# neyuru/RayTracing

Measured on AMD Instinct MI355X. Metric: ray-steps/sec (whole node) on vert_heterogeneous, 1M rays; % HBM roofline, higher is better.
Workload: dtype f64

## Files before the change

raytracing_amd/csrc/rtmi.hip:

```cpp
#include <hip/hip_runtime.h>

#include <chrono>
#include <cmath>
#include <cstdio>
#include <cstdlib>
#include <algorithm>
#include <cstring>
#include <exception>
#include <mutex>
#include <numeric>
#include <new>
#include <string>
#include <thread>
#include <utility>
#include <vector>

#include "rt_device.h"
#include "rtmi_field.h"

static thread_local std::string g_err;
static int fail(int code, const std::string& msg) {
    g_err = msg;
    return code;
}
// ... 212 lines not shown
template <typename T> __device__ __forceinline__ void derive_rt(const BatchDev<T>& a, rt::Ray<T>& r) {
    if (a.iso) rt::derive<T, true>(a.K, r); else rt::derive<T, false>(a.K, r);
}
template <> __device__ __forceinline__ void derive_rt<double>(const BatchDev<double>& a, rt::Ray<double>& r) {
    if (a.exact) rt::ex::derive(a.K, r);
    else if (a.iso) rt::derive<double, true>(a.K, r);
    else rt::derive<double, false>(a.K, r);
}
template <typename T> using InitGather = rt::PolyGather<T, rt::kPolyLane>;
template <typename T> __device__ __forceinline__ void n_gradient_rt(const BatchDev<T>& a, T x, T y, T& n, T& gx, T& gy) {
    InitGather<T> gg;
    rt::n_gradient(a.F, gg, true, x, y, n, gx, gy);
}
template <> __device__ __forceinline__ void n_gradient_rt<double>(const BatchDev<double>& a, double x, double y, double& n, double& gx, double& gy) {
    if (a.exact) { rt::GlobalGather<double> gg; rt::ex::n_gradient(a.F, gg, true, x, y, n, gx, gy); }
    else { InitGather<double> gg; rt::n_gradient(a.F, gg, true, x, y, n, gx, gy); }
}

template <typename T> __device__ __forceinline__ void init_ray(const BatchDev<T>& a, long k) {
    rt::Ray<T> r;
    r.x = a.x0[k]; r.y = a.y0[k]; r.th = a.th0[k];
    n_gradient_rt(a, (T)r.x, (T)r.y, r.n, r.gx, r.gy);
    derive_rt(a, r);
    r.dsim = 0; r.dreal = 0; r.tt = 0;
    a.acc(0)[k] = r.x; a.acc(1)[k] = r.y; a.acc(2)[k] = r.th; a.aux(0)[k] = r.n; a.aux(1)[k] = r.gx; a.aux(2)[k] = r.gy;
    a.acc(3)[k] = 0; a.acc(4)[k] = 0; a.acc(5)[k] = 0;
    if (a.has_hist) { a.aux(3)[k] = 0; a.aux(4)[k] = 0; a.aux(5)[k] = 0; a.aux(6)[k] = 0; }
    if (a.rot) { a.unit(0)[k] = r.ux; a.unit(1)[k] = r.uy; }
    if (a.hov) a.hov[k] = 0.f;
    a.istep[k] = 0;
    a.alive[k] = max_size_of(a, k) > 1;
    if (a.stride && a.rec_rows > 0) write_row(a, 0, k, r);
}
template <typename T> __global__ void k_init(BatchDev<T> a) {
    const long k = (long)blockIdx.x * blockDim.x + threadIdx.x;
    if (k >= a.R) return;
    init_ray(a, k);
}

__device__ __forceinline__ unsigned long long wave_sum(unsigned long long v) {
#pragma unroll
    for (int o = 32; o > 0; o >>= 1) v += __shfl_xor(v, o, 64);
    return v;
}

__global__ void k_stats(const int* istep, const unsigned char* alive, long R, unsigned long long* counters) {
    unsigned long long steps = 0, live = 0;
    for (long k = (long)blockIdx.x * blockDim.x + threadIdx.x; k < R; k += (long)gridDim.x * blockDim.x) {
        steps += (unsigned long long)istep[k];
        live += alive[k];
    }
    steps = wave_sum(steps);
    live = wave_sum(live);
    if ((threadIdx.x & 63) == 0) {
        if (steps) atomicAdd(&counters[0], steps);
        if (live) atomicAdd(&counters[1], live);
    }
}

template <bool COH, typename V> __device__ __forceinline__ V ld_state(const V* p) {
    if constexpr (COH) return __hip_atomic_load(p, __ATOMIC_RELAXED, __HIP_MEMORY_SCOPE_AGENT);
    else return *p;
}
template <bool COH, typename V> __device__ __forceinline__ void st_state(V* p, V v) {
    if constexpr (COH) __hip_atomic_store(p, v, __ATOMIC_RELAXED, __HIP_MEMORY_SCOPE_AGENT);
    else *p = v;
}
template <typename T, int METHOD, bool ISO, bool COH = false, bool HOV = false>
__device__ __forceinline__ void load_ray(const BatchDev<T>& a, long k, rt::Ray<T>& r, int& i) {
    r.x = ld_state<COH>(a.acc(0) + k); r.y = ld_state<COH>(a.acc(1) + k); r.th = ld_state<COH>(a.acc(2) + k);
// ... 455 lines not shown
    int flavour = kOrdinary;
    int slot() const { return (iso ? 1 : 0) | (lds ? 2 : 0) | flat << 2 | flavour << 4; }
    bool operator==(const StepBuild& o) const { return dtype == o.dtype && ki == o.ki && slot() == o.slot(); }
};
struct rtmi_batch {
    const rtmi_field* field = nullptr;
    rtmi_params p{};
    int64_t R = 0;
    size_t esz = 8;
    hipStream_t stream = nullptr;
    void* state = nullptr;
    int* istep = nullptr;
    unsigned char* alive = nullptr;
    void *s_ray = nullptr, *n_ray = nullptr;
    bool own_s = false, own_n = false;
    double* launch = nullptr;
    int* perm = nullptr;
    void *vstep = nullptr, *vstep2h = nullptr;
    int* vmax = nullptr;
    unsigned long long* counters = nullptr;
    unsigned long long* h_counters = nullptr;
    std::vector<std::pair<hipEvent_t, hipEvent_t>> events;
    size_t ev_used = 0;
    size_t pass_ev_start = 0;
    double kernel_ms = 0;
    double total_kernel_ms = 0;
    uint64_t total_launches = 0;
    uint32_t launches = 0;
    int persistent_blocks = 0;
    int sliced_blocks = 0;
    unsigned long long* sliced_ctl = nullptr;
    bool dirty = false;
    bool dirty_state = false;
    bool state_rows = false;
    double auto_ms[2][RTMI_AUTO_SAMPLES] = {{0, 0, 0}, {0, 0, 0}};
    int auto_n[2] = {0, 0};
    int auto_kept = -1;
    double gold_sup[8] = {0, 0, 0, 0, 0, 0, 0, 0};
    int lat_simds = 0;
    int mode_used = RTMI_LAUNCH_PLAIN;
    const void* kfn_used = nullptr;
    uint32_t auto_fallbacks = 0;
    void* staging = nullptr;
    size_t staging_bytes = 0;
    hipGraph_t graph = nullptr;
    hipGraphExec_t graph_exec = nullptr;
    StepBuild graph_build;
    int graph_nsteps = 0, graph_count = 0, graph_block = 0;
    struct Retrace* rt = nullptr;
    bool is_retrace_sub = false;
};
static void drop_graph(rtmi_batch* b);

struct Retrace {
    rtmi_batch* sub = nullptr;
    unsigned cap = 0;
    unsigned long long* rq = nullptr;
    unsigned* host_count = nullptr;
    float* hov = nullptr;
    static constexpr int kAux = 4;
    hipStream_t aux[kAux] = {nullptr, nullptr, nullptr, nullptr};
    hipEvent_t ev_main = nullptr, ev_aux[kAux] = {nullptr, nullptr, nullptr, nullptr};
    hipStream_t masked = nullptr;
    hipEvent_t ev_in = nullptr, ev_out = nullptr;
    unsigned chunks = 0;
    unsigned launched = 0;
    unsigned scattered = 0;
    bool pending = false;
    unsigned long long* dbg = nullptr;
    unsigned overflow = 0;
    double* org = nullptr;
    int* org_istep = nullptr;
    bool from_set = false;
    unsigned swept = 0;
    uint64_t total = 0;
    unsigned rot = 0;
    bool rot_learned = false;
};
static int retrace_create(rtmi_batch* b, const double* x0, const double* y0, const double* theta0);
static void retrace_destroy(rtmi_batch* b);
static int retrace_reset(rtmi_batch* b);
static int retrace_drain(rtmi_batch* b, bool overlap);
static bool retrace_wanted(const rtmi_batch* b);
#define RETRACE_FLUSH(b)                                             \
    do {                                                             \
        if ((b)->rt && (b)->rt->pending) {                           \
            const int rcf_ = retrace_drain((b), false);              \
            if (rcf_) return rcf_;                                   \
        }                                                            \
    } while (0)

static int batch_staging(rtmi_batch* b, size_t bytes, void** out) {
    if (bytes > b->staging_bytes) {
        HIP_TRY(hipStreamSynchronize(b->stream));
        (void)hipFree(b->staging);
        b->staging = nullptr; b->staging_bytes = 0;
        hipError_t e = hipMalloc(&b->staging, bytes);
        if (e != hipSuccess) return fail(RTMI_ERR_ALLOC, std::string("staging buffer: ") + hipGetErrorString(e));
        b->staging_bytes = bytes;
    }
    *out = b->staging;
    return RTMI_OK;
}

constexpr long kWindowMinRays = 131072;
static bool window_loses(const rtmi_batch* b) {
    const int m = b->p.method;
    if (m != 5 && m != 9 && m != 10 && m != 11) return false;
    const rtmi_field* f = b->field;
    return std::fabs(b->p.step) > 0.5 * std::fmin(f->hx, f->hy);
}
template <typename T> static BatchDev<T> batch_dev(const rtmi_batch* b) {
    BatchDev<T> a;
    a.F = field_dev<T>(b->field, b->p.exact_basis);
    a.F.window = (b->p.field_path == 3 || (b->p.field_path == 0 && b->R >= kWindowMinRays && !window_loses(b))) ? 1 : 0;
    const rtmi_params& p = b->p;
    a.K.step = (T)p.step;
    a.K.step2h = (T)(libm_square(p.step) / 2.0);
    a.K.step2 = (T)libm_square(p.step);
    a.K.gamma = (T)p.gamma; a.K.g2m1 = (T)(p.gamma * p.gamma - 1.0);
    a.K.gamma_s = (T)p.gamma_step; a.K.g2m1_s = (T)(p.gamma_step * p.gamma_step - 1.0);
// ... 138 lines not shown
}

template <typename T, typename F> static hipError_t with_step_node_t(const rtmi_batch* b, const StepBuild& k, int sched, int nsteps, F&& use) {
    BatchDev<T> a = batch_dev<T>(b);
    int refill_min = b->p.refill_min > 0 ? b->p.refill_min : 32, chunk = 16;
    unsigned long long capacity = 0, timeout = 0, *ctl = b->sliced_ctl;
    void* plain[] = {&a, &nsteps};
    void* refill[] = {&a, &refill_min, &chunk};
    void* sliced[] = {&a, &nsteps, &capacity, &ctl, &timeout};
    const long bundles = (b->R + 255) / 256;
    hipKernelNodeParams kp{};
    kp.func = const_cast<void*>(step_kernel(k, sched));
    kp.blockDim = dim3(256);
    if (sched == RTMI_LAUNCH_PLAIN) {
        const int bs = b->p.block_size > 0 ? b->p.block_size : 256;
        kp.gridDim = dim3((unsigned)((b->R + bs - 1) / bs));
        kp.blockDim = dim3(bs);
        kp.kernelParams = plain;
    } else if (sched == RTMI_LAUNCH_SLICED) {
        capacity = sliced_capacity(b, nsteps);
        timeout = sliced_timeout_ticks(b, nsteps);
        kp.gridDim = dim3((unsigned)(bundles < b->sliced_blocks ? bundles : b->sliced_blocks));
        kp.kernelParams = sliced;
    } else {
        kp.gridDim = dim3((unsigned)(bundles < b->persistent_blocks ? bundles : b->persistent_blocks));
        kp.kernelParams = refill;
    }
    return use(kp);
}
template <typename F> static hipError_t with_step_node(const rtmi_batch* b, const StepBuild& k, int sched, int nsteps, F&& use) {
    return by_dtype(k.dtype, [&](auto t) { return with_step_node_t<decltype(t)>(b, k, sched, nsteps, use); });
}

static int batch_init_state(rtmi_batch* b, bool clear_traj) {
    hipStream_t st = b->stream;
    const size_t R = (size_t)b->R;
    HIP_TRY(hipMemsetAsync(b->counters, 0, 4 * sizeof(unsigned long long), st));
    if (b->rt) { const int rcr = retrace_reset(b); if (rcr) return rcr; }
    if (clear_traj && b->s_ray) HIP_TRY(hipMemsetAsync(b->s_ray, 0, (size_t)b->p.rec_rows * 6 * R * b->esz, st));
    if (clear_traj && b->n_ray) HIP_TRY(hipMemsetAsync(b->n_ray, 0, (size_t)b->p.rec_rows * R * b->esz, st));
    b->dirty = false;
    by_dtype(b->p.dtype, [&](auto t) { hipLaunchKernelGGL(k_init<decltype(t)>, blocks(b->R), dim3(256), 0, st, batch_dev<decltype(t)>(b)); });
    HIP_TRY(hipGetLastError());
    b->kernel_ms = 0; b->launches = 0; b->pass_ev_start = b->ev_used; b->dirty_state = false;
    b->state_rows = false;
    return RTMI_OK;
}

RTMI_EXPORT void rtmi_batch_destroy(rtmi_batch* b) {
    if (!b) return;
    (void)hipStreamSynchronize(b->stream);
    (void)hipFree(b->state); (void)hipFree(b->istep); (void)hipFree(b->alive); (void)hipFree(b->launch);
    (void)hipFree(b->perm);
    (void)hipFree(b->vstep); (void)hipFree(b->vstep2h); (void)hipFree(b->vmax);
    (void)hipFree(b->counters); (void)hipFree(b->sliced_ctl); (void)hipFree(b->staging);
    if (b->h_counters) (void)hipHostFree(b->h_counters);
    if (b->own_s) (void)hipFree(b->s_ray);
    if (b->own_n) (void)hipFree(b->n_ray);
    retrace_destroy(b);
    drop_graph(b);
    for (auto& e : b->events) { (void)hipEventDestroy(e.first); (void)hipEventDestroy(e.second); }
    delete b;
}

RTMI_EXPORT int rtmi_batch_create(const rtmi_field* f, const rtmi_params* p, int64_t R, const double* x0,
                                  const double* y0, const double* theta0, void* stream, rtmi_batch** out) {
    ARG_TRY(f && p && x0 && y0 && theta0 && out, "rtmi_batch_create: null argument");
    ARG_TRY(R > 0 && R < (1ll << 31), "rtmi_batch_create: R must be in [1, 2^31)");
    ARG_TRY(p->method >= RTMI_OP_MIN && p->method <= RTMI_OP_MAX, "rtmi_batch_create: method must be 1..11");
    ARG_TRY(p->dtype == f->dtype, "rtmi_batch_create: params.dtype differs from the field's dtype");
    ARG_TRY(p->step > 0 && std::isfinite(p->step), "rtmi_batch_create: step must be finite and > 0");
    ARG_TRY(p->gamma > 0 && p->gamma_step > 0, "rtmi_batch_create: gamma must be > 0");
    ARG_TRY(p->max_size >= 2, "rtmi_batch_create: max_size must be >= 2");
    ARG_TRY(p->method != 7 || p->max_size >= 4, "rtmi_batch_create: op7 needs max_size >= 4 (two bootstrap rows)");
    ARG_TRY(p->record_stride >= 0, "rtmi_batch_create: record_stride < 0");
    ARG_TRY(p->box[1] > p->box[0] && p->box[3] > p->box[2], "rtmi_batch_create: empty box");
    ARG_TRY(p->launch_mode >= RTMI_LAUNCH_AUTO && p->launch_mode <= RTMI_LAUNCH_PLAIN,
            "rtmi_batch_create: launch_mode must be 0 (auto), 1 (refill), 2 (sliced) or 3 (plain)");
    ARG_TRY(p->slice_steps >= 0, "rtmi_batch_create: slice_steps must be >= 0");
    ARG_TRY(p->refill_min >= 0 && p->refill_min <= 64, "rtmi_batch_create: refill_min must be in [0, 64]");
    ARG_TRY(p->exact_basis == 0 || p->exact_basis == 1, "rtmi_batch_create: exact_basis must be 0 or 1");
    ARG_TRY(p->field_path >= 0 && p->field_path <= 3, "rtmi_batch_create: field_path must be 0 (auto), 1 (global), 2 (wave-shared: LDS tile) or 3 (wave-shared: scalar cache)");
    ARG_TRY(p->sort_rays == 0 || p->sort_rays == 1, "rtmi_batch_create: sort_rays must be 0 or 1");
    ARG_TRY(p->lazy_clear == 0 || p->lazy_clear == 1, "rtmi_batch_create: lazy_clear must be 0 or 1");
    ARG_TRY(p->no_n_ray == 0 || p->no_n_ray == 1, "rtmi_batch_create: no_n_ray must be 0 or 1");
    ARG_TRY(!(p->no_n_ray && p->ext_n_ray), "rtmi_batch_create: no_n_ray set together with ext_n_ray");
    ARG_TRY(p->reference_order >= 0 && p->reference_order <= 3, "rtmi_batch_create: reference_order must be 0 .. 3 (RTMI_ORDER_*)");
    ARG_TRY(!(p->reference_order == RTMI_ORDER_REFERENCE && p->dtype != RTMI_F64), "rtmi_batch_create: reference_order 1 needs an fp64 batch (the reference has no fp32)");
    ARG_TRY(p->no_retrace == 0 || p->no_retrace == 1, "rtmi_batch_create: no_retrace must be 0 or 1");
    DEVICE_TRY(f, "rtmi_batch_create");
    rtmi_batch* b = new (std::nothrow) rtmi_batch();
    if (!b) return fail(RTMI_ERR_ALLOC, "rtmi_batch_create: host allocation failed");
    b->field = f; b->p = *p; b->R = R; b->esz = p->dtype == RTMI_F64 ? 8 : 4; b->stream = (hipStream_t)stream;
    if (p->method >= 10) gold_sup_derivatives(p->gamma_step, b->gold_sup);
    if (batch_exact(b) && (p->method == 1 || p->method == 4 || p->method == 7 || p->method == 8)) {
        const int rct = ensure_rcp14_table(b->stream);
        if (rct) { delete b; return rct; }
    }
    if (b->p.record_stride > 0 && b->p.rec_rows <= 0)
        b->p.rec_rows = ((int64_t)p->max_size + p->record_stride - 1) / p->record_stride;
    if (b->p.record_stride == 0) b->p.rec_rows = 0;
    int rc = RTMI_OK;
    auto body = [&]() -> int {
        const size_t Rz = (size_t)R;
        const int naux = p->method == 7 ? 7 : (rt::rotates_unit(p->method, p->dtype == RTMI_F64) && !ref_order(*p)) ? 5 : 3;
        HIP_TRY(hipMalloc(&b->state, 6 * Rz * sizeof(double) + naux * Rz * b->esz));
        HIP_TRY(hipMalloc(&b->istep, Rz * sizeof(int)));
        HIP_TRY(hipMalloc(&b->alive, Rz));
        HIP_TRY(hipMalloc(&b->launch, 3 * Rz * sizeof(double)));
        HIP_TRY(hipMalloc(&b->counters, 4 * sizeof(unsigned long long)));
        HIP_TRY(hipHostMalloc(&b->h_counters, 2 * sizeof(unsigned long long)));
        if (b->p.record_stride > 0) {
            if (p->ext_s_ray) b->s_ray = p->ext_s_ray;
            else { HIP_TRY(hipMalloc(&b->s_ray, (size_t)b->p.rec_rows * 6 * Rz * b->esz)); b->own_s = true; }
            if (p->no_n_ray) b->n_ray = nullptr;
            else if (p->ext_n_ray) b->n_ray = p->ext_n_ray;
            else { HIP_TRY(hipMalloc(&b->n_ray, (size_t)b->p.rec_rows * Rz * b->esz)); b->own_n = true; }
        }
        std::vector<double> sorted;
        if (p->sort_rays) {
            std::vector<int> perm(Rz);
            std::iota(perm.begin(), perm.end(), 0);
            const double ibx = 1.0 / (16.0 * f->hx), iby = 1.0 / (16.0 * f->hy);
            auto block = [&](int k) {
                const double u = (x0[k] - f->ax) * ibx, v = (y0[k] - f->ay) * iby;
                const long bu = u >= 0 && u < 65535 ? (long)u : (u < 0 ? -1 : 65535);
                const long bv = v >= 0 && v < 65535 ? (long)v : (v < 0 ? -1 : 65535);
                return bv * 65537 + bu;
            };
            std::vector<long> key(Rz);
            for (size_t k = 0; k < Rz; k++) key[k] = block((int)k);
            std::stable_sort(perm.begin(), perm.end(), [&](int i, int j) {
                if (key[i] != key[j]) return key[i] < key[j];
                const double a = theta0[i], c = theta0[j];
                if (a == a && c == c) return a < c;
                return a == a && c != c;
            });
            sorted.resize(3 * Rz);
            for (size_t k = 0; k < Rz; k++) {
                sorted[k] = x0[perm[k]]; sorted[Rz + k] = y0[perm[k]]; sorted[2 * Rz + k] = theta0[perm[k]];
            }
            HIP_TRY(hipMalloc(&b->perm, Rz * sizeof(int)));
            HIP_TRY(hipMemcpyAsync(b->perm, perm.data(), Rz * sizeof(int), hipMemcpyHostToDevice, b->stream));
            HIP_TRY(hipMemcpyAsync(b->launch, sorted.data(), 3 * Rz * 8, hipMemcpyHostToDevice, b->stream));
            HIP_TRY(hipStreamSynchronize(b->stream));
        } else {
            HIP_TRY(hipMemcpyAsync(b->launch, x0, Rz * 8, hipMemcpyHostToDevice, b->stream));
            HIP_TRY(hipMemcpyAsync(b->launch + Rz, y0, Rz * 8, hipMemcpyHostToDevice, b->stream));
            HIP_TRY(hipMemcpyAsync(b->launch + 2 * Rz, theta0, Rz * 8, hipMemcpyHostToDevice, b->stream));
        }
        HIP_TRY(hipStreamSynchronize(b->stream));
        int dev = 0, cus = 0, per_cu = 0;
        HIP_TRY(hipGetDevice(&dev));
        HIP_TRY(hipDeviceGetAttribute(&cus, hipDeviceAttributeMultiprocessorCount, dev));
        b->lat_simds = cus * 4;
        const StepBuild k = step_build(b);
        b->kfn_used = step_kernel(k, RTMI_LAUNCH_PLAIN);
        HIP_TRY(hipOccupancyMaxActiveBlocksPerMultiprocessor(&per_cu, step_kernel(k, RTMI_LAUNCH_REFILL), 256, 0));
        b->persistent_blocks = cus * (per_cu > 0 ? per_cu : 1);
        if (b->p.launch_mode == RTMI_LAUNCH_SLICED || b->p.launch_mode == RTMI_LAUNCH_AUTO) {
            HIP_TRY(hipOccupancyMaxActiveBlocksPerMultiprocessor(&per_cu, step_kernel(k, RTMI_LAUNCH_SLICED), 256, 0));
            b->sliced_blocks = cus * (per_cu > 0 ? per_cu : 1);
            if (getenv("RTMI_DEBUG")) fprintf(stderr, "rtmi: sliced kernel: %d CUs x %d resident blocks\n", cus, per_cu);
            if (b->p.launch_mode == RTMI_LAUNCH_SLICED)
                ARG_TRY(sliced_feasible(b),
                        "rtmi_batch_create: RTMI_LAUNCH_SLICED: slice_steps too small for this batch size and max_size (queue > 256 MB)");
            const bool may_slice = b->p.launch_mode == RTMI_LAUNCH_SLICED || (sliced_feasible(b) && (R + 255) / 256 > b->sliced_blocks);
            if (may_slice)
                HIP_TRY(hipMalloc(&b->sliced_ctl, (4 + sliced_capacity(b, sliced_steps(b))) * sizeof(unsigned long long)));
        }
        if (retrace_wanted(b)) {
            const int rcr = retrace_create(b, x0, y0, theta0);
            if (rcr) return rcr;
        }
        return batch_init_state(b, true);
    };
    try {
        rc = body();
    } catch (const std::exception& e) {
        rc = fail(RTMI_ERR_ALLOC, std::string("rtmi_batch_create: ") + e.what());
    }
    if (rc) { rtmi_batch_destroy(b); return rc; }
    *out = b;
    return RTMI_OK;
}

template <typename T>
__global__ void k_set_per_ray(BatchDev<T> a, const double* step, const double* step2h, const int* ms, T* vstep, T* vstep2h, int* vmax) {
    const long k = (long)blockIdx.x * blockDim.x + threadIdx.x;
    if (k >= a.R) return;
    const long o = out_index(a, k);
    vstep[k] = (T)step[o]; vstep2h[k] = (T)step2h[o]; vmax[k] = ms[o];
    a.alive[k] = a.istep[k] + 1 < ms[o];
}

RTMI_EXPORT int rtmi_batch_set_per_ray(rtmi_batch* b, const double* step, const int32_t* max_size) {
    ARG_TRY(b && step && max_size, "rtmi_batch_set_per_ray: null");
    ARG_TRY(b->p.launch_mode == RTMI_LAUNCH_PLAIN || b->p.launch_mode == RTMI_LAUNCH_AUTO,
            "rtmi_batch_set_per_ray: per-ray steps run on the one-lane-per-ray kernel (RTMI_LAUNCH_PLAIN or RTMI_LAUNCH_AUTO)");
    DEVICE_TRY(b->field, "rtmi_batch_set_per_ray");
    drop_graph(b);
    if (b->launches != 0 || b->dirty_state)
        return fail(RTMI_ERR_STATE, "rtmi_batch_set_per_ray: only valid on a fresh or reset batch (before any rtmi_step / rtmi_run / "
                                    "rtmi_batch_set_state): rays that already stopped would be revived");
    const size_t R = (size_t)b->R;
    std::vector<double> h2;
    try {
        h2.resize(R);
// ... 82 lines not shown
    if (b->perm) return fail(RTMI_ERR_STATE, "rtmi_internal_relaunch: not on a batch with sort_rays");
    ARG_TRY(!(max_size && b->p.launch_mode != RTMI_LAUNCH_PLAIN && b->p.launch_mode != RTMI_LAUNCH_AUTO),
            "rtmi_internal_relaunch: per-ray max_size runs on the one-lane-per-ray kernel (RTMI_LAUNCH_PLAIN or RTMI_LAUNCH_AUTO)");
    DEVICE_TRY(b->field, "rtmi_internal_relaunch");
    drop_graph(b);
    const size_t R = (size_t)b->R;
    HIP_TRY(hipStreamSynchronize(b->stream));
    HIP_TRY(hipMemcpyAsync(b->launch + 2 * R, theta0, R * sizeof(double), hipMemcpyDeviceToDevice, b->stream));
    if (max_size) {
        if (!b->vstep) {
            std::vector<double> h1, h2;
            std::vector<float> f1, f2;
            try {
                if (b->p.dtype == RTMI_F64) { h1.assign(R, b->p.step); h2.assign(R, libm_square(b->p.step) / 2.0); }
                else { f1.assign(R, (float)b->p.step); f2.assign(R, (float)(libm_square(b->p.step) / 2.0)); }
            } catch (const std::exception& e) {
                return fail(RTMI_ERR_ALLOC, std::string("rtmi_internal_relaunch: ") + e.what());
            }
            HIP_TRY(hipMalloc(&b->vstep, R * b->esz));
            HIP_TRY(hipMalloc(&b->vstep2h, R * b->esz));
            HIP_TRY(hipMalloc(&b->vmax, R * sizeof(int)));
            const void* p1 = b->p.dtype == RTMI_F64 ? (const void*)h1.data() : (const void*)f1.data();
            const void* p2 = b->p.dtype == RTMI_F64 ? (const void*)h2.data() : (const void*)f2.data();
            HIP_TRY(hipMemcpy(b->vstep, p1, R * b->esz, hipMemcpyHostToDevice));
            HIP_TRY(hipMemcpy(b->vstep2h, p2, R * b->esz, hipMemcpyHostToDevice));
        }
        HIP_TRY(hipMemcpyAsync(b->vmax, max_size, R * sizeof(int), hipMemcpyDeviceToDevice, b->stream));
    }
    b->dirty = true;
    return batch_init_state(b, true);
}

template <typename T> __global__ void k_set_state(BatchDev<T> a, const double* st, const double* hist, const int* istep, const unsigned char* live,
                                                  double* org, int* org_istep) {
    const long k = (long)blockIdx.x * blockDim.x + threadIdx.x;
    if (k >= a.R) return;
    const long o = out_index(a, k);
    a.acc(0)[k] = st[o]; a.acc(1)[k] = st[(size_t)a.R + o]; a.acc(2)[k] = st[(size_t)2 * a.R + o];
    for (int q = 0; q < 3; q++) a.aux(q)[k] = (T)st[(size_t)(3 + q) * a.R + o];
    for (int q = 0; q < 3; q++) a.acc(3 + q)[k] = st[(size_t)(6 + q) * a.R + o];
    if (a.has_hist && hist)
        for (int q = 0; q < 4; q++) a.aux(3 + q)[k] = (T)hist[(size_t)q * a.R + o];
    if (a.rot) {
        if (hist && live) {
            a.unit(0)[k] = (T)hist[o]; a.unit(1)[k] = (T)hist[(size_t)a.R + o];
        } else {
            T sn, cs;
            rt::M<T>::sincos_(a.acc(2)[k], &sn, &cs);
            a.unit(0)[k] = cs; a.unit(1)[k] = sn;
        }
    }
    if (a.hov) a.hov[k] = (a.rot && hist && live) ? (float)hist[(size_t)2 * a.R + o] : 0.f;
    if (istep) a.istep[k] = istep[o];
    if (org) {
        for (int q = 0; q < 9; q++) org[(size_t)q * a.R + k] = st[(size_t)q * a.R + o];
        org_istep[k] = a.istep[k];
    }
    a.alive[k] = (live ? live[o] != 0 : true) && a.istep[k] + 1 < max_size_of(a, k);
}
template <typename T> __global__ void k_get_state(BatchDev<T> a, double* out, int* oi, unsigned char* ol) {
    const long k = (long)blockIdx.x * blockDim.x + threadIdx.x;
    if (k >= a.R) return;
    const long o = out_index(a, k);
    const size_t R = (size_t)a.R;
    out[o] = a.acc(0)[k]; out[R + o] = a.acc(1)[k]; out[2 * R + o] = a.acc(2)[k];
    for (int q = 0; q < 3; q++) out[(3 + q) * R + o] = (double)a.aux(q)[k];
    for (int q = 0; q < 3; q++) out[(6 + q) * R + o] = a.acc(3 + q)[k];
    double h[4] = {0, 0, 0, 0};
    if (a.has_hist) for (int q = 0; q < 4; q++) h[q] = (double)a.aux(3 + q)[k];
    else if (a.rot) { h[0] = (double)a.unit(0)[k]; h[1] = (double)a.unit(1)[k]; h[2] = a.hov ? (double)a.hov[k] : 0.0; }
    for (int q = 0; q < 4; q++) out[(9 + q) * R + o] = h[q];
    oi[o] = a.istep[k];
    ol[o] = a.alive[k];
}

static int set_state_impl(rtmi_batch* b, const double* state9, const double* hist4, const int32_t* istep, const uint8_t* live, const char* who) {
    ARG_TRY(b && state9, std::string(who) + ": null");
    DEVICE_TRY(b->field, who);
    const size_t R = (size_t)b->R;
    double* org = nullptr;
    int* org_istep = nullptr;
    if (b->rt) {
        Retrace* t = b->rt;
        const int rcr = retrace_reset(b);
        if (rcr) return rcr;
        if (!live) {
            if (!t->org) {
                HIP_TRY(hipMalloc(&t->org, 9 * R * sizeof(double) + R * sizeof(int)));
                t->org_istep = (int*)(t->org + 9 * R);
            }
            org = t->org; org_istep = t->org_istep;
        }
    }
    b->dirty = true;
    b->dirty_state = true;
    b->state_rows = istep ? std::any_of(istep, istep + R, [](int32_t i) { return i != 0; }) : (b->state_rows || b->launches != 0);
    void* stg = nullptr;
    int rc = batch_staging(b, 13 * R * sizeof(double) + R * sizeof(int) + R, &stg);
    if (rc) return rc;
    double* d = (double*)stg;
    int* di = (int*)(d + 13 * R);
    unsigned char* dl = (unsigned char*)(di + R);
    hipError_t e = hipMemcpyAsync(d, state9, 9 * R * 8, hipMemcpyHostToDevice, b->stream);
    if (e == hipSuccess && hist4) e = hipMemcpyAsync(d + 9 * R, hist4, 4 * R * 8, hipMemcpyHostToDevice, b->stream);
    if (e == hipSuccess && istep) e = hipMemcpyAsync(di, istep, R * sizeof(int), hipMemcpyHostToDevice, b->stream);
    if (e == hipSuccess && live) e = hipMemcpyAsync(dl, live, R, hipMemcpyHostToDevice, b->stream);
    if (e == hipSuccess) {
        by_dtype(b->p.dtype, [&](auto t) {
            hipLaunchKernelGGL(k_set_state<decltype(t)>, blocks(b->R), dim3(256), 0, b->stream, batch_dev<decltype(t)>(b), d, hist4 ? d + 9 * R : nullptr,
                               istep ? di : nullptr, live ? dl : nullptr, org, org_istep);
        });
        e = hipGetLastError();
    }
    if (e == hipSuccess) e = hipStreamSynchronize(b->stream);
    if (e != hipSuccess) return fail(RTMI_ERR_HIP, std::string(who) + ": " + hipGetErrorString(e));
    if (org) b->rt->from_set = true;
    return RTMI_OK;
}
RTMI_EXPORT int rtmi_batch_set_state(rtmi_batch* b, const double* state9, const double* hist4, const int32_t* istep) {
    return set_state_impl(b, state9, hist4, istep, nullptr, "rtmi_batch_set_state");
}
RTMI_EXPORT int rtmi_batch_restore_state(rtmi_batch* b, const double* state9, const double* aux4, const int32_t* istep, const uint8_t* alive) {
    ARG_TRY(aux4 && istep && alive, "rtmi_batch_restore_state: null (pass what rtmi_batch_get_state returned)");
    return set_state_impl(b, state9, aux4, istep, alive, "rtmi_batch_restore_state");
}

RTMI_EXPORT int rtmi_batch_get_state(rtmi_batch* b, double* state9, double* hist4, int32_t* istep, uint8_t* alive) {
    ARG_TRY(b, "rtmi_batch_get_state: null");
    DEVICE_TRY(b->field, "rtmi_batch_get_state");
    RETRACE_FLUSH(b);
    const size_t R = (size_t)b->R;
    void* stg = nullptr;
    int rc = batch_staging(b, 13 * R * sizeof(double) + R * sizeof(int) + R, &stg);
    if (rc) return rc;
    double* d = (double*)stg;
    int* di = (int*)(d + 13 * R);
    unsigned char* dl = (unsigned char*)(di + R);
    by_dtype(b->p.dtype, [&](auto t) { hipLaunchKernelGGL(k_get_state<decltype(t)>, blocks(b->R), dim3(256), 0, b->stream, batch_dev<decltype(t)>(b), d, di, dl); });
    hipError_t e = hipGetLastError();
    if (e == hipSuccess && state9) e = hipMemcpyAsync(state9, d, 9 * R * 8, hipMemcpyDeviceToHost, b->stream);
    if (e == hipSuccess && hist4) e = hipMemcpyAsync(hist4, d + 9 * R, 4 * R * 8, hipMemcpyDeviceToHost, b->stream);
    if (e == hipSuccess && istep) e = hipMemcpyAsync(istep, di, R * sizeof(int), hipMemcpyDeviceToHost, b->stream);
    if (e == hipSuccess && alive) e = hipMemcpyAsync(alive, dl, R, hipMemcpyDeviceToHost, b->stream);
// ... 40 lines not shown
static void drop_graph(rtmi_batch* b) {
    if (b->graph_exec) (void)hipGraphExecDestroy(b->graph_exec);
    if (b->graph) (void)hipGraphDestroy(b->graph);
    b->graph_exec = nullptr; b->graph = nullptr; b->graph_nsteps = b->graph_count = 0;
}
static hipError_t build_step_graph(rtmi_batch* b, const StepBuild& k, int nsteps, int count, int bs) {
    drop_graph(b);
    hipError_t e = hipGraphCreate(&b->graph, 0);
    if (e != hipSuccess) return e;
    e = with_step_node(b, k, RTMI_LAUNCH_PLAIN, nsteps, [&](const hipKernelNodeParams& kp) {
        hipGraphNode_t prev = nullptr;
        for (int i = 0; i < count; i++) {
            hipGraphNode_t node = nullptr;
            const hipError_t en = hipGraphAddKernelNode(&node, b->graph, prev ? &prev : nullptr, prev ? 1 : 0, &kp);
            if (en != hipSuccess) return en;
            prev = node;
        }
        return hipSuccess;
    });
    if (e != hipSuccess) return e;
    e = hipGraphInstantiate(&b->graph_exec, b->graph, nullptr, nullptr, 0);
    if (e != hipSuccess) return e;
    b->graph_build = k; b->graph_nsteps = nsteps; b->graph_count = count; b->graph_block = bs;
    return hipSuccess;
}

RTMI_EXPORT int rtmi_step_repeat(rtmi_batch* b, int32_t nsteps, int32_t count) {
    ARG_TRY(b, "rtmi_step_repeat: null");
    ARG_TRY(nsteps > 0 && count > 0 && count <= 65536, "rtmi_step_repeat: nsteps must be > 0 and count in 1..65536");
    DEVICE_TRY(b->field, "rtmi_step_repeat");
    ARG_TRY(b->p.block_size == 0 || (b->p.block_size % 64 == 0 && b->p.block_size <= 256),
            "rtmi_step_repeat: block_size must be a multiple of 64, at most 256");
    const int bs = b->p.block_size > 0 ? b->p.block_size : 256;
    const StepBuild k = step_build(b);
    if (!b->graph_exec || !(b->graph_build == k) || b->graph_nsteps != nsteps || b->graph_count != count || b->graph_block != bs) {
        const hipError_t e = build_step_graph(b, k, nsteps, count, bs);
        if (e != hipSuccess) {
            drop_graph(b);
            (void)hipGetLastError();
            for (int i = 0; i < count; i++) { const int rc = rtmi_step(b, nsteps); if (rc) return rc; }
            return RTMI_OK;
        }
    }
    std::pair<hipEvent_t, hipEvent_t>* evp = nullptr;
    int rc0 = next_event_pair(b, &evp);
    if (rc0) return rc0;
    HIP_TRY(hipEventRecord(evp->first, b->stream));
    HIP_TRY(hipGraphLaunch(b->graph_exec, b->stream));
    if (b->rt) b->rt->pending = true;
    HIP_TRY(hipEventRecord(evp->second, b->stream));
    b->launches += (uint32_t)count; b->total_launches += (uint64_t)count;
    b->mode_used = RTMI_LAUNCH_PLAIN;
    b->kfn_used = step_kernel(k, RTMI_LAUNCH_PLAIN);
    return RTMI_OK;
}

struct OwnStream {
    rtmi_batch* b = nullptr;
    hipStream_t callers = nullptr;
    bool on = false;
    int enter(rtmi_batch* b_);
    int leave();
    ~OwnStream() { if (on) b->stream = callers; }
};

int OwnStream::enter(rtmi_batch* b_) {
// ... 17 lines not shown

static int timed_launch(rtmi_batch* b, int sched, int nsteps, bool drain, std::pair<hipEvent_t, hipEvent_t>** evp) {
    int rc = next_event_pair(b, evp);
    if (rc) return rc;
    auto* ev = *evp;
    if (sched == RTMI_LAUNCH_SLICED) HIP_TRY(hipMemsetAsync(b->sliced_ctl, 0, (4 + sliced_capacity(b, nsteps)) * sizeof(unsigned long long), b->stream));
    if (sched == RTMI_LAUNCH_REFILL) HIP_TRY(hipMemsetAsync(b->counters + 2, 0, sizeof(unsigned long long), b->stream));
    HIP_TRY(hipEventRecord(ev->first, b->stream));
    OwnStream own;
    if (drain) { const int rco = own.enter(b); if (rco) return rco; }
    (void)with_step_node(b, step_build(b), sched, nsteps, [&](const hipKernelNodeParams& kp) {
        b->kfn_used = kp.func;
        return hipLaunchKernel(kp.func, kp.gridDim, kp.blockDim, kp.kernelParams, 0, b->stream);
    });
    HIP_TRY(hipGetLastError());
    if (b->rt) {
        b->rt->pending = true;
        if (drain) { const int rcd = retrace_drain(b, true); if (rcd) return rcd; }
    }
    { const int rco = own.leave(); if (rco) return rco; }
    HIP_TRY(hipEventRecord(ev->second, b->stream));
    b->launches++; b->total_launches++;
    b->mode_used = sched;
    return RTMI_OK;
}

static int step_impl(rtmi_batch* b, int32_t nsteps, bool drain) {
    ARG_TRY(b, "rtmi_step: null");
    ARG_TRY(nsteps > 0, "rtmi_step: nsteps must be > 0");
    DEVICE_TRY(b->field, "rtmi_step");
    ARG_TRY(b->p.block_size == 0 || (b->p.block_size % 64 == 0 && b->p.block_size <= 256),
            "rtmi_step: block_size must be a multiple of 64, at most 256");
    std::pair<hipEvent_t, hipEvent_t>* evp = nullptr;
    return timed_launch(b, RTMI_LAUNCH_PLAIN, nsteps, drain, &evp);
}
RTMI_EXPORT int rtmi_step(rtmi_batch* b, int32_t nsteps) { return step_impl(b, nsteps, false); }

static int read_counters(rtmi_batch* b) {
    HIP_TRY(hipMemsetAsync(b->counters, 0, 2 * sizeof(unsigned long long), b->stream));
    hipLaunchKernelGGL(k_stats, dim3(256), dim3(256), 0, b->stream, b->istep, b->alive, (long)b->R, b->counters);
    HIP_TRY(hipGetLastError());
    HIP_TRY(hipMemcpyAsync(b->h_counters, b->counters, 2 * sizeof(unsigned long long), hipMemcpyDeviceToHost, b->stream));
    HIP_TRY(hipStreamSynchronize(b->stream));
    return RTMI_OK;
}

static bool sliced_ready(const rtmi_batch* b) { return b->sliced_ctl && !b->vstep && uniform_rows_ok(b); }

static int run_sliced(rtmi_batch* b, std::pair<hipEvent_t, hipEvent_t>** evp) {
    int rc = timed_launch(b, RTMI_LAUNCH_SLICED, sliced_steps(b), true, evp);
    if (rc) return rc;
    rc = read_counters(b);
    if (rc) return rc;
    if (b->h_counters[1] != 0) {
        unsigned long long ctl4[4] = {0, 0, 0, 0};
        HIP_TRY(hipMemcpy(ctl4, b->sliced_ctl, sizeof(ctl4), hipMemcpyDeviceToHost));
        return fail(RTMI_ERR_STATE, ctl4[3] == 1 ? "rtmi_run: the sliced launch abandoned a wait for a queue entry"
                                  : ctl4[3] == 2 ? "rtmi_run: the sliced launch ran out of queue entries"
                                                 : "rtmi_run: rays still live after the sliced launch");
    }
    return RTMI_OK;
}

static int run_plain(rtmi_batch* b, std::pair<hipEvent_t, hipEvent_t>** evp) {
    int rc = step_impl(b, b->p.max_size, true);
    if (rc) return rc;
    *evp = &b->events[b->ev_used - 1];
    rc = read_counters(b);
    if (rc) return rc;
    if (b->h_counters[1] != 0) return fail(RTMI_ERR_STATE, "rtmi_run: rays still live after a full-length launch");
    return RTMI_OK;
}


static bool retrace_wanted(const rtmi_batch* b) {
    const rtmi_params& p = b->p;
    return !b->is_retrace_sub && !p.no_retrace && p.dtype == RTMI_F64 && b->field->steep_cells > 0 &&
           (p.reference_order == RTMI_ORDER_DEFAULT || p.reference_order == RTMI_ORDER_FAST_FIELD) &&
           rt::rotates_unit(p.method, true);
}
static unsigned retrace_capacity(int64_t R) {
    const int64_t c = std::min<int64_t>(std::max<int64_t>((R / 128 + 63) / 64 * 64, 1024), 65536);
    return (unsigned)std::min<int64_t>(c, (R + 63) / 64 * 64);
}
constexpr int kRetraceOut = 256;
constexpr int kRetraceCus = 8;
template <int METHOD>
__global__ __launch_bounds__(64, 3) void k_retrace_ref(BatchDev<double> s, BatchDev<double> m, const unsigned long long* rq, unsigned lo, unsigned hi,
                                                       int marked_only, unsigned long long* dbg, const double* org, const int* org_istep) {
    typedef double T;
    __builtin_amdgcn_s_setprio(3);
    const unsigned j = lo + blockIdx.x * blockDim.x + threadIdx.x;
    const bool valid = j < hi && (!marked_only || s.alive[j < hi ? j : lo] == 2);
    const unsigned long long e = valid ? rq[1 + j] : 0ull;
    long k = (long)(e & 0xffffffffull);
    if (k >= m.R) k = 0;
    rt::Consts<T> K = m.K;
    int max_size = m.max_size;
    if (m.vstep) { K.step = m.vstep[k]; K.step2h = m.vstep2h[k]; K.step2 = K.step2h * 2.0; max_size = m.vmax[k]; }
    const int ref_until = marked_only ? 0x7fffffff : (int)(e >> 32);
// ... 370 lines not shown
            HIP_TRY(hipMemset(t->dbg, 0, 8 * sizeof(unsigned long long)));
            fprintf(stderr, "rtmi: retrace: %u rays: %llu reference-order steps (at most %llu per ray), %llu fused steps, longest ray %llu steps, %llu hovered again\n", n, h[0], h[3], h[1], h[4], h[2]);
        }
    }
    if (evp) HIP_TRY(hipEventRecord(evp->second, b->stream));
    t->pending = false;
    return RTMI_OK;
}

#define RTMI_AUTO_RUNS (2 * RTMI_AUTO_SAMPLES)
static int auto_next(const int n[2]) {
    static const int order[RTMI_AUTO_RUNS] = {0, 1, 1, 0, 0, 1};
    const int k = n[0] + n[1];
    return k < RTMI_AUTO_RUNS ? order[k] : -1;
}
static double auto_median(const double* v, int n) {
    double a[RTMI_AUTO_SAMPLES];
    for (int i = 0; i < n; i++) a[i] = v[i];
    std::sort(a, a + n);
    return n == 0 ? 1e30 : (n & 1) ? a[n / 2] : 0.5 * (a[n / 2 - 1] + a[n / 2]);
}
static int auto_decide(const double* sliced_ms, int ns, const double* plain_ms, int np) {
    return auto_median(plain_ms, np) < 0.97 * auto_median(sliced_ms, ns) ? RTMI_LAUNCH_PLAIN : RTMI_LAUNCH_SLICED;
}

RTMI_EXPORT int rtmi_run(rtmi_batch* b) {
    ARG_TRY(b, "rtmi_run: null");
    DEVICE_TRY(b->field, "rtmi_run");
    int rc;
    std::pair<hipEvent_t, hipEvent_t>* ev = nullptr;
    if (b->p.launch_mode == RTMI_LAUNCH_REFILL) {
        rc = timed_launch(b, RTMI_LAUNCH_REFILL, 0, true, &ev);
        if (rc) return rc;
        return read_counters(b);
    }
    if (b->p.launch_mode == RTMI_LAUNCH_SLICED) return sliced_ready(b) ? run_sliced(b, &ev) : run_plain(b, &ev);
    if (b->p.launch_mode == RTMI_LAUNCH_PLAIN || !sliced_ready(b)) return run_plain(b, &ev);
    const bool fresh = b->launches == 0 && !b->dirty_state;
    int pick = b->auto_kept >= 0 ? b->auto_kept : auto_next(b->auto_n);
    const bool exploring = b->auto_kept < 0;
    rc = pick == 0 ? run_sliced(b, &ev) : run_plain(b, &ev);
    if (rc == RTMI_ERR_STATE && pick == 0) {
        b->auto_kept = 1;
        b->auto_fallbacks++;
        if (getenv("RTMI_DEBUG")) fprintf(stderr, "rtmi: RTMI_LAUNCH_AUTO: the sliced launch gave up a wait (%s); finishing with the plain kernel\n", g_err.c_str());
        return run_plain(b, &ev);
    }
    if (rc == RTMI_OK && exploring && fresh && ev) {
        float ms = 0;
        if (hipEventElapsedTime(&ms, ev->first, ev->second) == hipSuccess) {
            b->auto_ms[pick][b->auto_n[pick]++] = (double)ms;
            if (auto_next(b->auto_n) < 0) {
                b->auto_kept = auto_decide(b->auto_ms[0], b->auto_n[0], b->auto_ms[1], b->auto_n[1]) == RTMI_LAUNCH_PLAIN ? 1 : 0;
                if (getenv("RTMI_DEBUG"))
                    fprintf(stderr, "rtmi: RTMI_LAUNCH_AUTO: sliced %.3f %.3f %.3f ms, plain %.3f %.3f %.3f ms -> %s\n", b->auto_ms[0][0], b->auto_ms[0][1],
                            b->auto_ms[0][2], b->auto_ms[1][0], b->auto_ms[1][1], b->auto_ms[1][2], b->auto_kept ? "plain" : "sliced");
            }
        }
    }
    return rc;
}

RTMI_EXPORT int rtmi_debug_auto_rule(const double* sliced_ms, int ns, const double* plain_ms, int np, int* next, int* decision) {
    ARG_TRY(ns >= 0 && np >= 0 && ns <= RTMI_AUTO_SAMPLES && np <= RTMI_AUTO_SAMPLES && (sliced_ms || ns == 0) && (plain_ms || np == 0),
            "rtmi_debug_auto_rule: at most RTMI_AUTO_SAMPLES samples per schedule");
    const int n[2] = {ns, np};
// ... 257 lines not shown
```

Baseline: 143.4 billion.

## Defer trajectory clearing to zero only rows not overwritten by the run

Replaces the full memset of the recorded trajectory buffers on reset with a per-ray high-water mark of written rows. After the run, a tail-zeroing kernel clears only rows beyond each ray's final step up to the previous high-water mark. This removes most of the bulk HBM write traffic of the clear. The cost is an extra per-ray int array, bookkeeping in init/set_state, and deferral logic across several entry points.

```diff
diff --git a/raytracing_amd/csrc/rtmi.hip b/raytracing_amd/csrc/rtmi.hip
--- a/raytracing_amd/csrc/rtmi.hip
+++ b/raytracing_amd/csrc/rtmi.hip
@@ -268,10 +268,49 @@
     a.alive[k] = max_size_of(a, k) > 1;
     if (a.stride && a.rec_rows > 0) write_row(a, 0, k, r);
 }
-template <typename T> __global__ void k_init(BatchDev<T> a) {
+__device__ __forceinline__ int rows_reached(int istep, int stride, long rec_rows) {
+    long r = (istep > 0 ? istep : 0) / stride;
+    r = r < rec_rows - 1 ? r : rec_rows - 1;
+    return (int)(r + 1);
+}
+__device__ __forceinline__ void fold_mark(int* hw, long k, int istep, int stride, long rec_rows) {
+    const int reached = rows_reached(istep, stride, rec_rows);
+    if (reached > hw[k]) hw[k] = reached;
+}
+template <typename T> __global__ void k_init(BatchDev<T> a, int* hw, int fresh) {
     const long k = (long)blockIdx.x * blockDim.x + threadIdx.x;
     if (k >= a.R) return;
+    if (hw) {
+        if (fresh) hw[k] = (int)a.rec_rows;
+        else fold_mark(hw, k, a.istep[k], a.stride, a.rec_rows);
+    }
     init_ray(a, k);
+}
+template <typename T> __global__ __launch_bounds__(256) void k_zero_tail(T* s_ray, T* n_ray, const int* istep, int* hw, long R, int stride, long rec_rows) {
+    const long k = (long)blockIdx.x * 256 + threadIdx.x;
+    const bool live = k < R;
+    int lo = 0x7fffffff, hi = 0;
+    if (live) {
+        lo = rows_reached(istep[k], stride, rec_rows);
+        hi = hw[k];
+        hi = (long)hi < rec_rows ? hi : (int)rec_rows;
+    }
+    int wlo = lo, whi = hi;
+#pragma unroll
+    for (int o = 32; o > 0; o >>= 1) {
+        const int l2 = __shfl_xor(wlo, o, 64), h2 = __shfl_xor(whi, o, 64);
+        wlo = l2 < wlo ? l2 : wlo; whi = h2 > whi ? h2 : whi;
+    }
+    const size_t Rz = (size_t)R;
+    for (long r = wlo; r < (long)whi; r++) {
+        if (r >= lo && r < hi) {
+            T* p = s_ray + (size_t)r * 6 * Rz + (size_t)k;
+#pragma unroll
+            for (int q = 0; q < 6; q++) __builtin_nontemporal_store(T(0), p + (size_t)q * Rz);
+            if (n_ray) __builtin_nontemporal_store(T(0), n_ray + (size_t)r * Rz + (size_t)k);
+        }
+    }
+    if (live) hw[k] = lo;
 }
 
 __device__ __forceinline__ unsigned long long wave_sum(unsigned long long v) {
@@ -793,6 +832,8 @@
     unsigned long long* sliced_ctl = nullptr;
     bool dirty = false;
     bool dirty_state = false;
+    int* hw = nullptr;
+    bool clear_pending = false;
     bool state_rows = false;
     double auto_ms[2][RTMI_AUTO_SAMPLES] = {{0, 0, 0}, {0, 0, 0}};
     int auto_n[2] = {0, 0};
@@ -843,11 +884,16 @@
 static int retrace_reset(rtmi_batch* b);
 static int retrace_drain(rtmi_batch* b, bool overlap);
 static bool retrace_wanted(const rtmi_batch* b);
+static int resolve_clear(rtmi_batch* b);
 #define RETRACE_FLUSH(b)                                             \
     do {                                                             \
         if ((b)->rt && (b)->rt->pending) {                           \
             const int rcf_ = retrace_drain((b), false);              \
             if (rcf_) return rcf_;                                   \
+        }                                                            \
+        if ((b)->clear_pending) {                                    \
+            const int rcc_ = resolve_clear((b));                     \
+            if (rcc_) return rcc_;                                   \
         }                                                            \
     } while (0)
 
@@ -1052,15 +1098,39 @@
     return by_dtype(k.dtype, [&](auto t) { return with_step_node_t<decltype(t)>(b, k, sched, nsteps, use); });
 }
 
-static int batch_init_state(rtmi_batch* b, bool clear_traj) {
+static int resolve_clear(rtmi_batch* b) {
+    if (!b->clear_pending) return RTMI_OK;
+    if (!b->s_ray || !b->hw) { b->clear_pending = false; return RTMI_OK; }
     hipStream_t st = b->stream;
-    const size_t R = (size_t)b->R;
+    hipStreamCaptureStatus cap = hipStreamCaptureStatusNone;
+    if (hipStreamIsCapturing(st, &cap) != hipSuccess) { (void)hipGetLastError(); cap = hipStreamCaptureStatusNone; }
+    if (cap != hipStreamCaptureStatusNone) return RTMI_OK;
+    by_dtype(b->p.dtype, [&](auto t) {
+        using T = decltype(t);
+        hipLaunchKernelGGL(k_zero_tail<T>, blocks(b->R), dim3(256), 0, st, (T*)b->s_ray, (T*)b->n_ray, (const int*)b->istep, b->hw, (long)b->R,
+                           (int)b->p.record_stride, (long)b->p.rec_rows);
+    });
+    HIP_TRY(hipGetLastError());
+    b->clear_pending = false;
+    return RTMI_OK;
+}
+
+static int batch_init_state(rtmi_batch* b, bool clear_traj, bool fresh = false) {
+    hipStream_t st = b->stream;
     HIP_TRY(hipMemsetAsync(b->counters, 0, 4 * sizeof(unsigned long long), st));
     if (b->rt) { const int rcr = retrace_reset(b); if (rcr) return rcr; }
-    if (clear_traj && b->s_ray) HIP_TRY(hipMemsetAsync(b->s_ray, 0, (size_t)b->p.rec_rows * 6 * R * b->esz, st));
-    if (clear_traj && b->n_ray) HIP_TRY(hipMemsetAsync(b->n_ray, 0, (size_t)b->p.rec_rows * R * b->esz, st));
+    if (clear_traj && b->s_ray) {
+        if (b->hw) b->clear_pending = true;
+        else {
+            const size_t R = (size_t)b->R;
+            HIP_TRY(hipMemsetAsync(b->s_ray, 0, (size_t)b->p.rec_rows * 6 * R * b->esz, st));
+            if (b->n_ray) HIP_TRY(hipMemsetAsync(b->n_ray, 0, (size_t)b->p.rec_rows * R * b->esz, st));
+        }
+    }
     b->dirty = false;
-    by_dtype(b->p.dtype, [&](auto t) { hipLaunchKernelGGL(k_init<decltype(t)>, blocks(b->R), dim3(256), 0, st, batch_dev<decltype(t)>(b)); });
+    by_dtype(b->p.dtype, [&](auto t) {
+        hipLaunchKernelGGL(k_init<decltype(t)>, blocks(b->R), dim3(256), 0, st, batch_dev<decltype(t)>(b), b->hw, fresh ? 1 : 0);
+    });
     HIP_TRY(hipGetLastError());
     b->kernel_ms = 0; b->launches = 0; b->pass_ev_start = b->ev_used; b->dirty_state = false;
     b->state_rows = false;
@@ -1071,7 +1141,7 @@
     if (!b) return;
     (void)hipStreamSynchronize(b->stream);
     (void)hipFree(b->state); (void)hipFree(b->istep); (void)hipFree(b->alive); (void)hipFree(b->launch);
-    (void)hipFree(b->perm);
+    (void)hipFree(b->perm); (void)hipFree(b->hw);
     (void)hipFree(b->vstep); (void)hipFree(b->vstep2h); (void)hipFree(b->vmax);
     (void)hipFree(b->counters); (void)hipFree(b->sliced_ctl); (void)hipFree(b->staging);
     if (b->h_counters) (void)hipHostFree(b->h_counters);
@@ -1136,6 +1206,7 @@
             if (p->no_n_ray) b->n_ray = nullptr;
             else if (p->ext_n_ray) b->n_ray = p->ext_n_ray;
             else { HIP_TRY(hipMalloc(&b->n_ray, (size_t)b->p.rec_rows * Rz * b->esz)); b->own_n = true; }
+            if (b->p.rec_rows > 0 && b->p.rec_rows < 0x7fffffff) HIP_TRY(hipMalloc(&b->hw, Rz * sizeof(int)));
         }
         std::vector<double> sorted;
         if (p->sort_rays) {
@@ -1193,7 +1264,7 @@
             const int rcr = retrace_create(b, x0, y0, theta0);
             if (rcr) return rcr;
         }
-        return batch_init_state(b, true);
+        return batch_init_state(b, true, true);
     };
     try {
         rc = body();
@@ -1342,7 +1413,7 @@
 }
 
 template <typename T> __global__ void k_set_state(BatchDev<T> a, const double* st, const double* hist, const int* istep, const unsigned char* live,
-                                                  double* org, int* org_istep) {
+                                                  double* org, int* org_istep, int* hw) {
     const long k = (long)blockIdx.x * blockDim.x + threadIdx.x;
     if (k >= a.R) return;
     const long o = out_index(a, k);
@@ -1361,7 +1432,10 @@
         }
     }
     if (a.hov) a.hov[k] = (a.rot && hist && live) ? (float)hist[(size_t)2 * a.R + o] : 0.f;
-    if (istep) a.istep[k] = istep[o];
+    if (istep) {
+        if (hw) fold_mark(hw, k, a.istep[k], a.stride, a.rec_rows);
+        a.istep[k] = istep[o];
+    }
     if (org) {
         for (int q = 0; q < 9; q++) org[(size_t)q * a.R + k] = st[(size_t)q * a.R + o];
         org_istep[k] = a.istep[k];
@@ -1402,6 +1476,7 @@
             org = t->org; org_istep = t->org_istep;
         }
     }
+    { const int rcc = resolve_clear(b); if (rcc) return rcc; }
     b->dirty = true;
     b->dirty_state = true;
     b->state_rows = istep ? std::any_of(istep, istep + R, [](int32_t i) { return i != 0; }) : (b->state_rows || b->launches != 0);
@@ -1418,7 +1493,7 @@
     if (e == hipSuccess) {
         by_dtype(b->p.dtype, [&](auto t) {
             hipLaunchKernelGGL(k_set_state<decltype(t)>, blocks(b->R), dim3(256), 0, b->stream, batch_dev<decltype(t)>(b), d, hist4 ? d + 9 * R : nullptr,
-                               istep ? di : nullptr, live ? dl : nullptr, org, org_istep);
+                               istep ? di : nullptr, live ? dl : nullptr, org, org_istep, b->hw);
         });
         e = hipGetLastError();
     }
@@ -1525,6 +1600,7 @@
     ARG_TRY(b->p.block_size == 0 || (b->p.block_size % 64 == 0 && b->p.block_size <= 256),
             "rtmi_step_repeat: block_size must be a multiple of 64, at most 256");
     const int bs = b->p.block_size > 0 ? b->p.block_size : 256;
+    { const int rcc = resolve_clear(b); if (rcc) return rcc; }
     const StepBuild k = step_build(b);
     if (!b->graph_exec || !(b->graph_build == k) || b->graph_nsteps != nsteps || b->graph_count != count || b->graph_block != bs) {
         const hipError_t e = build_step_graph(b, k, nsteps, count, bs);
@@ -1608,6 +1684,7 @@
     ARG_TRY(b->p.block_size == 0 || (b->p.block_size % 64 == 0 && b->p.block_size <= 256),
             "rtmi_step: block_size must be a multiple of 64, at most 256");
     std::pair<hipEvent_t, hipEvent_t>* evp = nullptr;
+    if (!drain) { const int rcc = resolve_clear(b); if (rcc) return rcc; }
     return timed_launch(b, RTMI_LAUNCH_PLAIN, nsteps, drain, &evp);
 }
 RTMI_EXPORT int rtmi_step(rtmi_batch* b, int32_t nsteps) { return step_impl(b, nsteps, false); }
@@ -1625,6 +1702,8 @@
 
 static int run_sliced(rtmi_batch* b, std::pair<hipEvent_t, hipEvent_t>** evp) {
     int rc = timed_launch(b, RTMI_LAUNCH_SLICED, sliced_steps(b), true, evp);
+    if (rc) return rc;
+    rc = resolve_clear(b);
     if (rc) return rc;
     rc = read_counters(b);
     if (rc) return rc;
@@ -1642,6 +1721,8 @@
     int rc = step_impl(b, b->p.max_size, true);
     if (rc) return rc;
     *evp = &b->events[b->ev_used - 1];
+    rc = resolve_clear(b);
+    if (rc) return rc;
     rc = read_counters(b);
     if (rc) return rc;
     if (b->h_counters[1] != 0) return fail(RTMI_ERR_STATE, "rtmi_run: rays still live after a full-length launch");
@@ -2078,6 +2159,8 @@
     if (b->p.launch_mode == RTMI_LAUNCH_REFILL) {
         rc = timed_launch(b, RTMI_LAUNCH_REFILL, 0, true, &ev);
         if (rc) return rc;
+        rc = resolve_clear(b);
+        if (rc) return rc;
         return read_counters(b);
     }
     if (b->p.launch_mode == RTMI_LAUNCH_SLICED) return sliced_ready(b) ? run_sliced(b, &ev) : run_plain(b, &ev);
```

After: 130.6 billion. 0.911x the previous value.
